# marlbenchmark/off-policy

Hardware: NVIDIA B200
Metric: learner grad-steps/sec (higher is better)
Workload: dtype f32

## Files before the change

### off-policy_b200/csrc/agent_bwd.cu

```cuda
#include "mx_internal.h"
#include "mx_kernels.h"
#include "mx_tile.cuh"
#include "mx_mma.cuh"

static inline size_t qhead_bwd_smem(int A) { return (size_t)(A * MX_H * 9 + 8 * 32 + 2 * 8 * MX_H + 2 * MX_H) * sizeof(float); }

__global__ void __launch_bounds__(256) k_qhead_bwd(QHeadBwdArgs a) {
  MX_DYN_SMEM(smem);
  const int tid = threadIdx.x, lane = tid & 31, warp = tid >> 5;
  const int A = a.A, AW = A * MX_H;
  float* wq_s = smem;
  float* dw_w = wq_s + AW;
  float* db_w = dw_w + 8 * AW;
  float* dg_w = db_w + 8 * 32;
  float* dbt_w = dg_w + 8 * MX_H;
  float* lg_s = dbt_w + 8 * MX_H;
  float* lb_s = lg_s + MX_H;
  for (int i = tid; i < AW; i += blockDim.x) wq_s[i] = a.theta[a.wq + i];
  for (int i = tid; i < 8 * AW + 8 * 32; i += blockDim.x) dw_w[i] = 0.f;
  for (int i = tid; i < MX_H; i += blockDim.x) { lg_s[i] = a.theta[a.lno_g + i]; lb_s[i] = a.theta[a.lno_b + i]; }
  MX_PDL_WAIT();
  __syncthreads();
  const int wglobal = blockIdx.x * (blockDim.x >> 5) + warp;
  const int wtotal = gridDim.x * (blockDim.x >> 5);
// ... 162 lines not shown
      dgh_s[cur][r][sq * MX_H + k] = vs;
      if (dg_on[r]) *dgp[r] = vg;
      dgp[r] -= dg_stride;
      cz[r] = dh * zg;
    }
    mx_cp_wait<PF - 1>();
    __syncthreads();
#pragma unroll
    for (int r = 0; r < RPC; ++r) {
      float2 p0 = make_float2(0.f, 0.f), p1 = p0, p2 = p0;
#pragma unroll
      for (int m = 0; m < 12; m += 3) {
        const float4 d0 = mx_ld4(&dgh_s[cur][r][16 * m + 4 * s]);
        const float4 d1 = mx_ld4(&dgh_s[cur][r][16 * (m + 1) + 4 * s]);
        const float4 d2 = mx_ld4(&dgh_s[cur][r][16 * (m + 2) + 4 * s]);
        p0 = mx_ffma2(w[2 * m], make_float2(d0.x, d0.y), p0); p0 = mx_ffma2(w[2 * m + 1], make_float2(d0.z, d0.w), p0);
        p1 = mx_ffma2(w[2 * m + 2], make_float2(d1.x, d1.y), p1); p1 = mx_ffma2(w[2 * m + 3], make_float2(d1.z, d1.w), p1);
        p2 = mx_ffma2(w[2 * m + 4], make_float2(d2.x, d2.y), p2); p2 = mx_ffma2(w[2 * m + 5], make_float2(d2.z, d2.w), p2);
      }
      p0 = mx_fadd2(mx_fadd2(p0, p1), p2);
      float p = p0.x + p0.y;
      p += __shfl_xor_sync(0xffffffffu, p, 1);
      p += __shfl_xor_sync(0xffffffffu, p, 2);
      carry[r] = cz[r] + p;
    }
  };
  int t = t_first;
  for (; t >= 1; t -= 2) { step(t, 0); step(t - 1, 1); }
  if (t == 0) step(0, 0);
  mx_cp_wait<0>();
}

#define BWD2_THREADS 128
template <int ROWS>
__global__ void __launch_bounds__(BWD2_THREADS, 2) k_gru_bwd2(GruBwdArgs a) {
  constexpr int RING = 8, PF = 6;
  __shared__ __align__(16) float ops_s[RING][ROWS][6][MX_H];
  __shared__ __align__(16) float dgh_s[2][ROWS][MX_G];
  const int tid = threadIdx.x;
  const int kp = tid >> 2, s = tid & 3;
  float2 w0[24], w1[24];
#pragma unroll
  for (int m = 0; m < 12; ++m)
#pragma unroll
    for (int c = 0; c < 2; ++c) {
      const int j = 16 * m + 4 * s + 2 * c;
      w0[2 * m + c] = make_float2(a.theta[a.whh + j * MX_H + 2 * kp], a.theta[a.whh + (j + 1) * MX_H + 2 * kp]);
      w1[2 * m + c] = make_float2(a.theta[a.whh + j * MX_H + 2 * kp + 1], a.theta[a.whh + (j + 1) * MX_H + 2 * kp + 1]);
    }
  const int T1 = a.T1 > 0 ? a.T1 : a.T + 1, N = a.N;
  MX_PDL_WAIT();
  const int t_first = a.T - 1;
  const bool pf_on = tid < 96;
  const int op = pf_on ? tid / 16 : 0, q4 = tid % 16;
  const bool pf_hprev = op == 4;
  const size_t pf_stride = (size_t)N * (op < 3 ? MX_G : MX_H);
  const int ku = 2 * kp + (s & 1);
  const int half = s >> 1;
  const size_t dg_stride = (size_t)N * MX_G;
  bool rok[ROWS];
  const float* pf_src[ROWS];
  const float* pf_h0[ROWS];
  float* dgp[ROWS];
  float carry[ROWS];
#pragma unroll
  for (int r = 0; r < ROWS; ++r) {
    const int row = blockIdx.x * ROWS + r;
    rok[r] = row < a.R;
    const int rr = rok[r] ? row : 0;
    const size_t m0 = ((size_t)(rr / N) * T1) * N + (rr % N);
    const float* base = op < 3 ? a.gates + m0 * MX_G + op * MX_H + 4 * q4 : (op == 3 ? a.hn : (op == 4 ? a.hall : a.dh_out)) + m0 * MX_H + 4 * q4;
    pf_src[r] = base + (ptrdiff_t)(pf_hprev ? t_first - 1 : t_first) * (ptrdiff_t)pf_stride;
    pf_h0[r] = (pf_hprev && a.h0) ? a.h0 + (size_t)rr * MX_H + 4 * q4 : nullptr;
    if (rok[r])
      for (int tz = a.T; tz < T1; ++tz)
        for (int c = tid; c < MX_G; c += BWD2_THREADS) a.dgi[(m0 + (size_t)tz * N) * MX_G + c] = 0.f;
    dgp[r] = a.dgi + (m0 + (size_t)t_first * N) * MX_G + ku;
    carry[r] = 0.f;
  }
  float* pf_dst = &ops_s[0][0][op][4 * q4];
  auto prefetch = [&](int t) {
    if (t >= 0 && pf_on) {
      const bool first = pf_hprev && t == 0;
#pragma unroll
      for (int r = 0; r < ROWS; ++r) {
        if (rok[r]) mx_cp16z(pf_dst + ((t & (RING - 1)) * ROWS + r) * (6 * MX_H), first ? (pf_h0[r] ? pf_h0[r] : a.hall) : pf_src[r], (first && !pf_h0[r]) ? 0 : 16);
        pf_src[r] -= pf_stride;
      }
    }
    mx_cp_commit();
  };
  if (ROWS > 1) {
    for (int idx = tid; idx < RING * ROWS * 6 * MX_H; idx += BWD2_THREADS) (&ops_s[0][0][0][0])[idx] = 0.f;
    __syncthreads();
  }
#pragma unroll
  for (int d = 0; d < PF; ++d) prefetch(t_first - d);
  mx_cp_wait<PF - 1>();
  __syncthreads();

  auto step = [&](const int t, const int cur) {
    prefetch(t - PF);
    float cz[ROWS];
#pragma unroll
    for (int r = 0; r < ROWS; ++r) {
      const float* o = &ops_s[t & (RING - 1)][r][0][0];
      const float rg = o[ku], zg = o[MX_H + ku], ng = o[2 * MX_H + ku], hn = o[3 * MX_H + ku], hp = o[4 * MX_H + ku];
      const float dh = o[5 * MX_H + ku] + carry[r];
      const float d_n = dh * (1.f - zg) * (1.f - ng * ng);
      const float d_z = dh * (hp - ng) * zg * (1.f - zg);
      const float d_r = d_n * hn * rg * (1.f - rg);
      dgh_s[cur][r][(half ? 2 * MX_H : 0) + ku] = half ? d_n * rg : d_r;
      if (!half) dgh_s[cur][r][MX_H + ku] = d_z;
      if (rok[r]) {
        dgp[r][half ? 2 * MX_H : 0] = half ? d_n : d_r;
        if (!half) dgp[r][MX_H] = d_z;
      }
      dgp[r] -= dg_stride;
      cz[r] = dh * zg;
    }
    mx_cp_wait<PF - 1>();
    __syncthreads();
#pragma unroll
    for (int r = 0; r < ROWS; ++r) {
      float2 a0 = make_float2(0.f, 0.f), a1 = a0, b0 = a0, b1 = a0;
#pragma unroll
      for (int m = 0; m < 12; ++m) {
        const float4 d = mx_ld4(&dgh_s[cur][r][16 * m + 4 * s]);
        const float2 lo = make_float2(d.x, d.y), hi = make_float2(d.z, d.w);
        a0 = mx_ffma2(w0[2 * m], lo, a0); b0 = mx_ffma2(w1[2 * m], lo, b0);
        a1 = mx_ffma2(w0[2 * m + 1], hi, a1); b1 = mx_ffma2(w1[2 * m + 1], hi, b1);
      }
      a0 = mx_fadd2(a0, a1); b0 = mx_fadd2(b0, b1);
      float p0 = a0.x + a0.y, p1 = b0.x + b0.y;
      p0 += __shfl_xor_sync(0xffffffffu, p0, 1); p1 += __shfl_xor_sync(0xffffffffu, p1, 1);
      p0 += __shfl_xor_sync(0xffffffffu, p0, 2); p1 += __shfl_xor_sync(0xffffffffu, p1, 2);
      carry[r] = cz[r] + ((s & 1) ? p1 : p0);
    }
  };
  int t = t_first;
  for (; t >= 1; t -= 2) { step(t, 0); step(t - 1, 1); }
  if (t == 0) step(0, 0);
  mx_cp_wait<0>();
}

struct FrontBwdSmem {
  int ldi, ld64, ldg;
  int o_dgi, o_dgn, o_x, o_hp, o_u, o_da, o_x0, o_xh0, o_dx0, o_wc, o_col, o_stat, o_lnp, total;
};
static FrontBwdSmem front_bwd_smem(int in_dim, int TM, bool gru_ext = false) {
  FrontBwdSmem s;
  const int I64 = mx_round_up(in_dim, 64);
  s.ldi = mx_ld(I64); s.ld64 = mx_ld(64); s.ldg = mx_ld(MX_G);
  int o = 0;
  s.o_dgi = o; o += TM * s.ldg;
  s.o_dgn = o; o += gru_ext ? 0 : TM * s.ld64;
  s.o_x = o; o += TM * s.ld64;
  s.o_hp = o; o += gru_ext ? 0 : TM * s.ld64;
  s.o_u = o; o += TM * s.ld64;
  s.o_da = o; o += TM * s.ld64;
  s.o_x0 = o; o += TM * s.ldi;
  s.o_xh0 = o; o += TM * s.ldi;
  s.o_dx0 = o; o += TM * s.ldi;
  s.o_wc = o; o += 64 * s.ld64;
  s.o_col = o; o += 2 * I64 + 4 * 64;
  s.o_stat = o; o += 3 * TM * 2;
  s.o_lnp = o; o += 4 * 64;
  s.total = o;
  return s;
}

template <int RM>
MX_DEVINL void ln64_bwd_relu(bool act_tanh, float (&v)[RM][4], const float* u_s, int ld, const float* stat , const float* gamma_s,
                             float (&dg)[4], float (&db)[4]) {
  const int tx = threadIdx.x & 15, ty = threadIdx.x >> 4;
#pragma unroll
// ... 380 lines not shown
        const float xs[8] = {x0.x, x0.y, x0.z, x0.w, x1.x, x1.y, x1.z, x1.w};
        const float2 d0 = *reinterpret_cast<const float2*>(dgi_s + r * sm.ldg + 2 * tn);
        const float2 d1 = *reinterpret_cast<const float2*>(dgi_s + r * sm.ldg + MX_H + 2 * tn);
        const float2 d2 = *reinterpret_cast<const float2*>(D2_s + r * ld2);
#pragma unroll
        for (int k = 0; k < 8; ++k) {
          const float2 xx = make_float2(xs[k], xs[k]);
          acc[0][k] = mx_ffma2(d0, xx, acc[0][k]);
          acc[1][k] = mx_ffma2(d1, xx, acc[1][k]);
          acc[2][k] = mx_ffma2(d2, xx, acc[2][k]);
        }
      }
      float* W = gp + (pass ? L.whh : L.wih);
#pragma unroll
      for (int g = 0; g < 3; ++g)
#pragma unroll
        for (int h = 0; h < 2; ++h) {
          float* w = W + (size_t)(64 * g + 2 * tn + h) * MX_H + 8 * tk;
          float4 lo = make_float4(h ? acc[g][0].y : acc[g][0].x, h ? acc[g][1].y : acc[g][1].x, h ? acc[g][2].y : acc[g][2].x, h ? acc[g][3].y : acc[g][3].x);
          float4 hi = make_float4(h ? acc[g][4].y : acc[g][4].x, h ? acc[g][5].y : acc[g][5].x, h ? acc[g][6].y : acc[g][6].x, h ? acc[g][7].y : acc[g][7].x);
          if (accum) {
            const float4 p0 = mx_ld4(w), p1 = mx_ld4(w + 4);
            lo.x += p0.x; lo.y += p0.y; lo.z += p0.z; lo.w += p0.w; hi.x += p1.x; hi.y += p1.y; hi.z += p1.z; hi.w += p1.w;
          }
          mx_st4(w, lo); mx_st4(w + 4, hi);
        }
    }
    mx_colsum(dgi_s, sm.ldg, TM, MX_G, gp + L.bih, accum);
    mx_colsum(dgi_s, sm.ldg, TM, 2 * MX_H, gp + L.bhh, accum);
    mx_colsum(dgn_s, sm.ld64, TM, MX_H, gp + L.bhh + 2 * MX_H, accum);
  }
}

int mx_launch_qhead_bwd(const QHeadBwdArgs& a, int* nparts_used, cudaStream_t s) {
  int grid = mx_ceil_div(a.M, 8 * 4);
  const int cap = mx_num_sms();
  if (grid > cap) grid = cap;
  if (grid < 1) grid = 1;
  const size_t smem = qhead_bwd_smem(a.A);
#if !MX_EMU
  static size_t configured = 0;
  if (smem > 48 * 1024 && smem > configured) {
    if (cudaFuncSetAttribute(k_qhead_bwd, cudaFuncAttributeMaxDynamicSharedMemorySize, (int)smem) != cudaSuccess) { mx_set_error("qhead_bwd: smem %zu too large", smem); return 1; }
    configured = smem;
  }
#endif
  MX_LAUNCH_PDL(k_qhead_bwd, dim3(grid), dim3(256), smem, s, a);
  MX_COUNT();
  MX_MARK("k_qhead_bwd", s);
  *nparts_used = grid;
  return MX_CHECK_LAUNCH("qhead_bwd");
}

__global__ void __launch_bounds__(256) k_mlp_dgi(const float* __restrict__ dq_taken, const int32_t* __restrict__ act_idx, int ld_tn,
                                                 float* __restrict__ dgi, int B, int N) {
  const long long total = (long long)B * 2 * N * MX_G;
  MX_PDL_WAIT();
  for (long long i = (long long)blockIdx.x * blockDim.x + threadIdx.x; i < total; i += (long long)gridDim.x * blockDim.x) {
    const int c = (int)(i % MX_G);
    const long long m = i / MX_G;
    const int n = (int)(m % N);
    const long long bt = m / N;
    const int t = (int)(bt & 1);
    const long long b = bt >> 1;
    float v = 0.f;
    if (t == 0 && c == act_idx[b * ld_tn + n]) v = dq_taken[b * N + n];
// ... 88 lines not shown
  else rc = front_bwd_launch<2, false>(a, nparts_used, s);
  if (rc || !a.wgrad_external) return rc;
  return mx_launch_wgrad_tc(a, *nparts_used, s);
}

bool mx_wgrad_tc_usable(const FrontBwdArgs& a);
bool mx_gru_wgrad_split_usable(const FrontBwdArgs& a) {
  if (!g_mx_gru_wgrad_split || g_mx_front_bwd_mma || a.no_gru || a.skip_wgrad) return false;
  return !mx_front_bwd_tc_usable(a) && !mx_wgrad_tc_usable(a);
}
template <int RM>
static int gru_wgrad_launch(const FrontBwdArgs& a, cudaStream_t s) {
  const int TM = 16 * RM;
  GruWgradSmem sm = gru_wgrad_smem(TM);
  const size_t smem = (size_t)sm.total * sizeof(float) + 16;
  const int ntiles = mx_ceil_div(a.M, TM);
  int grid = mx_num_sms();
  if (grid > ntiles) grid = ntiles;
#if !MX_EMU
  static size_t configured = 0;
  if (smem > configured) { cudaFuncSetAttribute(k_gru_wgrad<RM>, cudaFuncAttributeMaxDynamicSharedMemorySize, (int)smem); configured = smem; }
#endif
  MX_LAUNCH_PDL(k_gru_wgrad<RM>, dim3(grid), dim3(MX_TILE_THREADS), smem, s, a, sm);
  MX_COUNT();
  MX_MARK("k_gru_wgrad", s);
  return MX_CHECK_LAUNCH("gru_wgrad");
}
int mx_launch_gru_wgrad(const FrontBwdArgs& a, cudaStream_t s) {
  const int rm = g_mx_front_bwd_rm ? g_mx_front_bwd_rm : front_bwd_pick_rm(a.M, a.L.in_dim, mx_num_sms(), true);
  if (rm == 3) return gru_wgrad_launch<3>(a, s);
  if (rm == 4) return gru_wgrad_launch<4>(a, s);
  return gru_wgrad_launch<2>(a, s);
}
```

### off-policy_b200/csrc/capi_common.cu

```cuda
#include <stdarg.h>
#include <stdio.h>
#include <string.h>

#include "mx_internal.h"

static thread_local char g_err[512] = "";
long long g_mx_launches = 0;
#if !MX_EMU
int g_mx_pdl = -1;
int g_mx_pdl_rows = 12288;
int g_mx_pdl_auto = 0;
int g_mx_pdl_skip_next = 0;
#endif

int g_mx_p2p_timeout_ms = 10000;
int g_mx_gru_rows = 1;
int g_mx_p2p_ll = 1;
int g_mx_mixer_split = 1;
int g_mx_mixer_split_rm = 0;
int g_mx_overlap = 1;
int g_mx_gru_threads = 0;
int g_mx_side_prio = 0;
int g_mx_hyper_late = 0;
int g_mx_mid_fused = 1;
int g_mx_gru_fwd_rpc = 0;
int g_mx_gru_bwd_rpc = 0;
int g_mx_overlap_rows = 1 << 20;
int mx_set_option_common(const char* name, int value) {
  if (!strcmp(name, "mixer_split")) { g_mx_mixer_split = value; return 0; }
  if (!strcmp(name, "mixer_split_rm")) { g_mx_mixer_split_rm = value; return 0; }
  if (!strcmp(name, "overlap")) { g_mx_overlap = value; return 0; }
  if (!strcmp(name, "overlap_rows")) { g_mx_overlap_rows = value; return 0; }
  if (!strcmp(name, "mid_fused")) { g_mx_mid_fused = value; return 0; }
  if (!strcmp(name, "optim_fused")) { g_mx_optim_fused = value; return 0; }
  if (!strcmp(name, "side_prio")) { g_mx_side_prio = value; return 0; }
  if (!strcmp(name, "hyper_late")) { g_mx_hyper_late = value; return 0; }
  if (!strcmp(name, "front_bwd_mma")) { g_mx_front_bwd_mma = value; return 0; }
  if (!strcmp(name, "gru_wgrad_split")) { g_mx_gru_wgrad_split = value; return 0; }
  if (!strcmp(name, "p2p_ll")) { g_mx_p2p_ll = value; return 0; }
  if (!strcmp(name, "gru_rows")) { g_mx_gru_rows = value; return 0; }
  if (!strcmp(name, "p2p_timeout_ms")) { g_mx_p2p_timeout_ms = value; return 0; }
#if !MX_EMU
  if (!strcmp(name, "smem_carveout")) { g_mx_smem_carveout = value; return 0; }
#else
  if (!strcmp(name, "smem_carveout")) return 0;
#endif
  if (!strcmp(name, "gather_tma")) { g_mx_gather_tma = value; return 0; }
  if (!strcmp(name, "gru_threads")) { g_mx_gru_threads = value; return 0; }
  if (!strcmp(name, "gru_fwd_rpc")) { g_mx_gru_fwd_rpc = value; return 0; }
  if (!strcmp(name, "gru_bwd_rpc")) { g_mx_gru_bwd_rpc = value; return 0; }
  return -1;
}

void mx_set_error(const char* fmt, ...) {
  va_list ap;
  va_start(ap, fmt);
  vsnprintf(g_err, sizeof(g_err), fmt, ap);
  va_end(ap);
}

extern "C" const char* mx_last_error(void) { return g_err; }
extern "C" int mx_abi_version(void) { return MX_ABI_VERSION; }

#define MX_MAX_FENCES 256
#if !MX_EMU
static cudaEvent_t g_fence[MX_MAX_FENCES];
static unsigned char g_fence_set[MX_MAX_FENCES];
#endif
static int g_fence_n = 0;
extern "C" int mx_host_fence_alloc(void) {
  if (g_fence_n >= MX_MAX_FENCES) { mx_set_error("mx_host_fence_alloc: out of fences"); return -1; }
// ... 141 lines not shown
```

### off-policy_b200/csrc/mx_common.cuh

```cuda
#pragma once
#include <stdint.h>

#ifdef MARL_EMU
#include "emu_runtime.h"
#define MX_EMU 1
#define MX_LAUNCH_PDL MX_LAUNCH
#define MX_PDL_WAIT() ((void)0)
#define MX_PDL_THETA_WRITTEN() ((void)0)
#else
#include <cuda_runtime.h>
#define MX_EMU 0
#define MX_LAUNCH(kern, grid, block, smem, stream, ...) kern<<<(grid), (block), (smem), (stream)>>>(__VA_ARGS__)

extern int g_mx_pdl, g_mx_pdl_auto, g_mx_pdl_rows;
extern int g_mx_pdl_skip_next;
#define MX_PDL_THETA_WRITTEN() (g_mx_pdl_skip_next = 1)
#define MX_PDL_WAIT()                                                     \
  do {                                                                    \
    asm volatile("griddepcontrol.wait;" ::: "memory");                    \
    asm volatile("griddepcontrol.launch_dependents;" ::: "memory");       \
  } while (0)
extern int g_mx_smem_carveout;
void mx_prefer_carveout(const void* kern);
template <typename... KArgs, typename... Args>
// ... 83 lines not shown
  unsigned sa = (unsigned)__cvta_generic_to_shared(sdst);
  asm volatile("cp.async.cg.shared.global [%0], [%1], 16;" ::"r"(sa), "l"(gsrc) : "memory");
#endif
}
MX_DEVINL void mx_cp16z(float* sdst, const float* gsrc, int nbytes) {
#if MX_EMU
  if (nbytes) *reinterpret_cast<float4*>(sdst) = *reinterpret_cast<const float4*>(gsrc);
  else *reinterpret_cast<float4*>(sdst) = float4{0.f, 0.f, 0.f, 0.f};
#else
  unsigned sa = (unsigned)__cvta_generic_to_shared(sdst);
  asm volatile("cp.async.cg.shared.global [%0], [%1], 16, %2;" ::"r"(sa), "l"(gsrc), "r"(nbytes) : "memory");
#endif
}
MX_DEVINL void mx_cp4(float* sdst, const float* gsrc) {
#if MX_EMU
  *sdst = *gsrc;
#else
  unsigned sa = (unsigned)__cvta_generic_to_shared(sdst);
  asm volatile("cp.async.ca.shared.global [%0], [%1], 4;" ::"r"(sa), "l"(gsrc) : "memory");
#endif
}
MX_DEVINL void mx_cp_commit() {
#if !MX_EMU
  asm volatile("cp.async.commit_group;" ::: "memory");
#endif
}
template <int N>
MX_DEVINL void mx_cp_wait() {
#if !MX_EMU
  asm volatile("cp.async.wait_group %0;" ::"n"(N) : "memory");
#endif
}

MX_DEVINL float mx_ex2(float x) {
#if MX_EMU
  return exp2f(x);
#else
  float r;
  asm("ex2.approx.ftz.f32 %0, %1;" : "=f"(r) : "f"(x));
  return r;
#endif
}
MX_DEVINL float mx_rcp(float x) {
#if MX_EMU
  return 1.0f / x;
#else
  float r;
  asm("rcp.approx.ftz.f32 %0, %1;" : "=f"(r) : "f"(x));
  return r;
#endif
}
MX_DEVINL float mx_sigmoid_fast(float x) { return mx_rcp(1.0f + mx_ex2(-1.4426950408889634f * x)); }
MX_DEVINL float mx_tanh_fast(float x) { return fmaf(2.0f, mx_rcp(1.0f + mx_ex2(-2.8853900817779268f * x)), -1.0f); }

MX_DEVINL float2 mx_ffma2(float2 a, float2 b, float2 c) {
#if MX_EMU
  return make_float2(fmaf(a.x, b.x, c.x), fmaf(a.y, b.y, c.y));
#else
  return __ffma2_rn(a, b, c);
#endif
}
MX_DEVINL float2 mx_fadd2(float2 a, float2 b) {
#if MX_EMU
  return make_float2(a.x + b.x, a.y + b.y);
#else
  return __fadd2_rn(a, b);
// ... 5 lines not shown
```

### off-policy_b200/csrc/mx_internal.h

```cpp
#pragma once
#include "../../include/marl_b200.h"
#include "mx_common.cuh"

#include <functional>
#include <string>

void mx_set_error(const char* fmt, ...);
extern long long g_mx_launches;
extern int g_mx_prof_on;
void mx_prof_mark(const char* name, cudaStream_t s);
extern int g_mx_mixer_split, g_mx_mixer_split_rm, g_mx_overlap, g_mx_overlap_rows, g_mx_mid_fused, g_mx_gru_fwd_rpc, g_mx_gru_bwd_rpc, g_mx_optim_fused, g_mx_gru_threads, g_mx_front_bwd_mma, g_mx_hyper_late, g_mx_side_prio, g_mx_gru_wgrad_split, g_mx_p2p_ll, g_mx_p2p_timeout_ms, g_mx_gru_rows;
int mx_set_option_common(const char* name, int value);
#define MX_COUNT() (++g_mx_launches)
#define MX_MARK(name, s) do { if (g_mx_prof_on) mx_prof_mark((name), (s)); } while (0)

#if MX_EMU
static inline int mx_num_sms() { return 4; }
#define MX_CHECK_LAUNCH(what) 0
#else
int mx_num_sms();
int mx_check_launch(const char* what);
#define MX_CHECK_LAUNCH(what) mx_check_launch(what)
#endif

struct mx_graph {
#if !MX_EMU
  cudaGraph_t graph = nullptr;
  cudaGraphExec_t exec = nullptr;
#endif
  std::function<int(void*)> seq;
  std::function<void()> after_launch;
  int n_kernels = 0;
};
int mx_graph_capture_seq(std::function<int(void*)> seq, std::function<void()> after_launch, void* stream, mx_graph** out);

struct MxReplayState {
  int32_t filled;
  int32_t cursor;
  int32_t rng_pos;
  int32_t pad;
  double max_priority;
  double reward_mean, reward_std;
  double per_beta;
};
// ... 90 lines not shown
```

### off-policy_b200/csrc/mx_kernels.h

```cpp
#pragma once
#include "mx_internal.h"

struct FrontFwdArgs {
  const float* X;
  int ldx, M;
  int feature_norm;
  const float* theta[2];
  MxNetLayout L;
  float* gi[2];
  float *u1, *u2;
  float *st0, *st1, *st2;
  const float* tc_img[2];
  int act_tanh;
};
size_t mx_tc_image_floats(int in_dim);
int mx_launch_tc_prep_weights(const float* const theta[2], const MxNetLayout& L, float* const img[2], int nets, cudaStream_t s);
size_t mx_front_fwd_smem(int in_dim, int RM);
int mx_launch_front_fwd(const FrontFwdArgs& a, int nets, cudaStream_t s);

int mx_launch_pack_prev_act(const float* obs, int obs_ld, const float* acts, int act_ld, float* X, int ldx, int B, int T, int N, int O, int A,
                            cudaStream_t s);

struct GruFwdArgs {
  const float* theta[2];
// ... 115 lines not shown
  const float* X;
  int ldx, M, T, N;
  int T1;
  const float* h0;
  int feature_norm;
  const float* theta;
  MxNetLayout L;
  const float *u1, *u2, *st0, *st1, *st2;
  const float* dgi;
  const float* gates;
  const float* hall;
  float* gpart;
  long long P;
  int no_gru;
  float* dX;
  int skip_wgrad;
  float *da2_out, *da1_out;
  int wgrad_external;
  int use_mma;
  float* tc_imgT;
  int tc_imgT_ready;
  int act_tanh;
  float* ln_part;
  int ln_part_rows;
  int gru_wgrad_ext;
};
bool mx_gru_wgrad_split_usable(const FrontBwdArgs& a);
int mx_launch_gru_wgrad(const FrontBwdArgs& a, cudaStream_t s);
int mx_launch_tc_prep_weights_T(const float* theta, const MxNetLayout& L, float* imgT, cudaStream_t s);
bool mx_tc_prep_T_wanted(int in_dim);
size_t mx_tc_imageT_floats(int in_dim);
int mx_launch_front_bwd(const FrontBwdArgs& a, int* nparts_used, cudaStream_t s);
int mx_launch_wgrad_tc(const FrontBwdArgs& a, int nparts, cudaStream_t s);
bool mx_wgrad_tc_usable(const FrontBwdArgs& a);

struct OptimArgs {
  float *theta, *theta_tgt, *adam_m, *adam_v;
  const float* gpart;
  float* grad;
  long long P;
  int seg_begin[4], seg_end[4], seg_parts[4], nseg;
  const float* spart;
  int spart_n;
  float* info;
  double* adam_t;
  const float* err;
  int B, T;
  float per_nu, per_eps;
  float* prio;
  float lr, beta1, beta2, eps, max_grad_norm, tau;
  int world_size;
  float* normpart;
  int normpart_n;
  int fuse_polyak;
  float weight_decay;
  unsigned* sync;
  int phase;
  float* p2p_blocks[16];
  unsigned long long p2p_timeout_ns;
  int p2p_ll;
  float* xstat;
  long long p2p_slot;
  int p2p_rank, p2p_world;
};
static inline int mx_grad_reduce_blocks(long long P) { return (int)((P + 255) / 256); }
int mx_launch_grad_reduce(const OptimArgs& a, cudaStream_t s);
// ... 5 lines not shown
```

### off-policy_b200/csrc/qmix.cu

```cuda
#include <stdio.h>
#include <string.h>

#include <string>
#include <vector>

#include "mx_internal.h"
#include "mx_kernels.h"

extern int g_mx_front_tc;
bool mx_front_tc_usable(int in_dim, bool have_image);

static int take(int& off, int n) { int o = off; off += mx_round_up(n, 4); return o; }

int mx_net_layout(int in_dim, int out_dim, int base, MxNetLayout* L) {
  const int H = MX_H;
  int o = base;
  L->in_dim = in_dim; L->out_dim = out_dim;
  L->fn_g = take(o, in_dim); L->fn_b = take(o, in_dim);
  L->w1 = take(o, H * in_dim); L->b1 = take(o, H); L->ln1_g = take(o, H); L->ln1_b = take(o, H);
  L->wh = take(o, H * H); L->bh = take(o, H); L->lnh_g = take(o, H); L->lnh_b = take(o, H);
  L->w2 = take(o, H * H); L->b2 = take(o, H); L->ln2_g = take(o, H); L->ln2_b = take(o, H);
  L->wih = take(o, 3 * H * H); L->whh = take(o, 3 * H * H); L->bih = take(o, 3 * H); L->bhh = take(o, 3 * H);
  L->lno_g = take(o, H); L->lno_b = take(o, H);
  L->wq = take(o, out_dim * H); L->bq = take(o, out_dim);
// ... 431 lines not shown
    parts[3] = parts[1];
#if !MX_EMU
    if (overlap) fork_to_side(q, q->ev_core, s);
#endif
    if (mx_launch_mix_hyper_bwd(mx, &parts[2], side)) return 1;
  } else {
    if (mx_launch_qhead(qh, s)) return 1;
    if (split) {
      if (!overlap) { if (mx_launch_mix_hyper_fwd(mx, s)) return 1; }
#if !MX_EMU
      else join_from_side(q, q->ev_hyper, s);
#endif
      if (mx_launch_mix_core(mx, &parts[3], s)) return 1;
#if !MX_EMU
      if (overlap) fork_to_side(q, q->ev_core, s);
#endif
      if (mx_launch_mix_hyper_bwd(mx, &parts[2], side)) return 1;
    } else {
      if (mx_launch_mixer(mx, &parts[2], s)) return 1;
      parts[3] = parts[2];
    }
    QHeadBwdArgs hb;
    memset(&hb, 0, sizeof(hb));
    hb.theta = q->theta; hb.wq = q->agent.wq; hb.bq = q->agent.bq; hb.lno_g = q->agent.lno_g; hb.lno_b = q->agent.lno_b;
    hb.hall = gf.hall[0]; hb.sto = qh.sto; hb.act_idx = b->act_idx; hb.dq_taken = mx.dq_taken;
    hb.M = M; hb.T = T; hb.N = N; hb.A = c.act_dim; hb.ld_tn = ld_tn; hb.dh_out = ws + W.dh_out; hb.gpart = mx.gpart; hb.P = q->P;
    if (mx_launch_qhead_bwd(hb, &parts[1], s)) return 1;
  }

  GruBwdArgs gb;
  memset(&gb, 0, sizeof(gb));
  gb.theta = q->theta; gb.whh = q->agent.whh; gb.hall = gf.hall[0]; gb.gates = gf.gates; gb.hn = gf.hn; gb.dh_out = ws + W.dh_out;
  gb.dgi = ws + W.dgi; gb.R = B * N; gb.T = T; gb.N = N;
  if (mx_launch_gru_bwd(gb, s)) return 1;

  FrontBwdArgs fb;
  memset(&fb, 0, sizeof(fb));
  fb.X = X; fb.ldx = ldx; fb.M = M; fb.T = T; fb.N = N; fb.feature_norm = c.no_feature_norm ? 0 : 1; fb.act_tanh = c.use_tanh;
  fb.theta = q->theta; fb.L = q->agent; fb.u1 = ff.u1; fb.u2 = ff.u2; fb.st0 = ff.st0; fb.st1 = ff.st1; fb.st2 = ff.st2;
  fb.dgi = gb.dgi; fb.gates = gf.gates; fb.hall = gf.hall[0]; fb.gpart = mx.gpart; fb.P = q->P;
  fb.ln_part = ws + W.lnpart; fb.ln_part_rows = 2 * q->npart;
  fb.da2_out = ws + W.da2; fb.da1_out = ws + W.da1; fb.tc_imgT = ws + W.tcimgT; fb.tc_imgT_ready = q->imgT_fresh; q->imgT_fresh = 0;
  const bool gsplit = mx_gru_wgrad_split_usable(fb);
  if (gsplit) {
    fb.gru_wgrad_ext = 1;
#if !MX_EMU
    if (overlap) fork_to_side(q, q->ev_gbwd, s);
#endif
    if (mx_launch_gru_wgrad(fb, side)) return 1;
  }
  if (mx_launch_front_bwd(fb, &parts[0], s)) return 1;

#if !MX_EMU
  if ((split || gsplit) && overlap) join_from_side(q, q->ev_hbwd, s);
#endif
  *oa = optim_args(q, B, parts);
  return 0;
}

extern "C" int mx_qmix_backward_only(mx_qmix* q, const mx_batch* b, void* stream) {
  OptimArgs o;
  if (backward_core(q, b, stream, &o)) return 1;
  return mx_launch_grad_reduce(o, (cudaStream_t)stream);
}

extern "C" int mx_qmix_apply_ex(mx_qmix* q, uint32_t flags, void* stream) {
  const int parts[4] = {0, 0, 0, 0};
  OptimArgs o = optim_args(q, q->cfg.max_batch, parts, true);
  o.fuse_polyak = (flags & MX_STEP_FUSE_SOFT_UPDATE) ? 1 : 0;
  return mx_launch_adam(o, (cudaStream_t)stream);
}
extern "C" int mx_qmix_apply(mx_qmix* q, void* stream) { return mx_qmix_apply_ex(q, 0, stream); }

extern "C" int mx_qmix_step_ex(mx_qmix* q, const mx_batch* b, uint32_t flags, void* stream) {
  OptimArgs o;
  if (backward_core(q, b, stream, &o)) return 1;
  if (q->cfg.world_size == 1 || q->p2p_world) {
    o.fuse_polyak = (flags & MX_STEP_FUSE_SOFT_UPDATE) ? 1 : 0;
    const int rc = mx_launch_optim_fused(o, (cudaStream_t)stream);
    if (rc >= 0) return rc;
  }
  if (mx_launch_grad_reduce(o, (cudaStream_t)stream)) return 1;
  if (q->cfg.world_size > 1) {
    if (!q->p2p_world) return 0;
// ... 95 lines not shown
```

Baseline: 5935.

## Fuse GRU backward recurrence with front backward via warp-specialized producer/consumer kernel

Adds a fused kernel where one 128-thread group runs the reverse GRU recurrence per row and writes gate gradients into a double-buffered shared-memory chunk. A 256-thread consumer group computes the input-side weight grads, LN backward and MLP backward on each 16-step chunk as it completes. The two groups coordinate through named barriers. This removes the dgi round trip through global memory and one launch, and overlaps the serial recurrence with the front backward work. The fused path needs one block per row with the row count at most the SM count, and it disables the side-stream wgrad split when it is taken.

```diff
diff --git a/off-policy_b200/csrc/agent_bwd.cu b/off-policy_b200/csrc/agent_bwd.cu
--- a/off-policy_b200/csrc/agent_bwd.cu
+++ b/off-policy_b200/csrc/agent_bwd.cu
@@ -218,14 +218,13 @@
 }
 
 #define BWD2_THREADS 128
-template <int ROWS>
-__global__ void __launch_bounds__(BWD2_THREADS, 2) k_gru_bwd2(GruBwdArgs a) {
-  constexpr int RING = 8, PF = 6;
-  __shared__ __align__(16) float ops_s[RING][ROWS][6][MX_H];
-  __shared__ __align__(16) float dgh_s[2][ROWS][MX_G];
-  const int tid = threadIdx.x;
+struct GruBwdNoHook {
+  MX_DEVINL void begin(int) const {}
+  MX_DEVINL void value(int, int, int, float, float, float) const {}
+  MX_DEVINL void end(int) const {}
+};
+MX_DEVINL void gru_bwd2_load_w(const GruBwdArgs& a, int tid, float2 (&w0)[24], float2 (&w1)[24]) {
   const int kp = tid >> 2, s = tid & 3;
-  float2 w0[24], w1[24];
 #pragma unroll
   for (int m = 0; m < 12; ++m)
 #pragma unroll
@@ -234,8 +233,13 @@
       w0[2 * m + c] = make_float2(a.theta[a.whh + j * MX_H + 2 * kp], a.theta[a.whh + (j + 1) * MX_H + 2 * kp]);
       w1[2 * m + c] = make_float2(a.theta[a.whh + j * MX_H + 2 * kp + 1], a.theta[a.whh + (j + 1) * MX_H + 2 * kp + 1]);
     }
+}
+template <int ROWS, class Sync, class Hook>
+MX_DEVINL void gru_bwd2_body(const GruBwdArgs& a, const int tid, const int row_base, const float2 (&w0)[24], const float2 (&w1)[24],
+                             float (*ops_s)[ROWS][6][MX_H], float (*dgh_s)[ROWS][MX_G], Sync sync, const Hook& hook) {
+  constexpr int RING = 8, PF = 6;
+  const int kp = tid >> 2, s = tid & 3;
   const int T1 = a.T1 > 0 ? a.T1 : a.T + 1, N = a.N;
-  MX_PDL_WAIT();
   const int t_first = a.T - 1;
   const bool pf_on = tid < 96;
   const int op = pf_on ? tid / 16 : 0, q4 = tid % 16;
@@ -251,7 +255,7 @@
   float carry[ROWS];
 #pragma unroll
   for (int r = 0; r < ROWS; ++r) {
-    const int row = blockIdx.x * ROWS + r;
+    const int row = row_base + r;
     rok[r] = row < a.R;
     const int rr = rok[r] ? row : 0;
     const size_t m0 = ((size_t)(rr / N) * T1) * N + (rr % N);
@@ -278,14 +282,15 @@
   };
   if (ROWS > 1) {
     for (int idx = tid; idx < RING * ROWS * 6 * MX_H; idx += BWD2_THREADS) (&ops_s[0][0][0][0])[idx] = 0.f;
-    __syncthreads();
+    sync();
   }
 #pragma unroll
   for (int d = 0; d < PF; ++d) prefetch(t_first - d);
   mx_cp_wait<PF - 1>();
-  __syncthreads();
+  sync();
 
   auto step = [&](const int t, const int cur) {
+    hook.begin(t);
     prefetch(t - PF);
     float cz[ROWS];
 #pragma unroll
@@ -302,11 +307,13 @@
         dgp[r][half ? 2 * MX_H : 0] = half ? d_n : d_r;
         if (!half) dgp[r][MX_H] = d_z;
       }
+      hook.value(t, ku, half, d_r, d_z, d_n);
       dgp[r] -= dg_stride;
       cz[r] = dh * zg;
     }
+    hook.end(t);
     mx_cp_wait<PF - 1>();
-    __syncthreads();
+    sync();
 #pragma unroll
     for (int r = 0; r < ROWS; ++r) {
       float2 a0 = make_float2(0.f, 0.f), a1 = a0, b0 = a0, b1 = a0;
@@ -328,6 +335,18 @@
   for (; t >= 1; t -= 2) { step(t, 0); step(t - 1, 1); }
   if (t == 0) step(0, 0);
   mx_cp_wait<0>();
+}
+
+struct BlockSync { MX_DEVINL void operator()() const { __syncthreads(); } };
+
+template <int ROWS>
+__global__ void __launch_bounds__(BWD2_THREADS, 2) k_gru_bwd2(GruBwdArgs a) {
+  __shared__ __align__(16) float ops_s[8][ROWS][6][MX_H];
+  __shared__ __align__(16) float dgh_s[2][ROWS][MX_G];
+  float2 w0[24], w1[24];
+  gru_bwd2_load_w(a, threadIdx.x, w0, w1);
+  MX_PDL_WAIT();
+  gru_bwd2_body<ROWS>(a, threadIdx.x, blockIdx.x * ROWS, w0, w1, ops_s, dgh_s, BlockSync(), GruBwdNoHook());
 }
 
 struct FrontBwdSmem {
@@ -774,6 +793,201 @@
   }
 }
 
+#define BF_CONSUMERS 256
+#define BF_THREADS (BF_CONSUMERS + BWD2_THREADS)
+#define BF_TC 16
+#define BF_BAR_REC 1
+#define BF_BAR_FRONT 2
+#define BF_BAR_FULL 3
+#define BF_BAR_EMPTY 5
+
+struct BwdFrontSmem { int ld64, ldg, o_dgi, o_wih, o_w2, o_w1, o_dgn, o_x, o_hp, o_u2, o_u1, o_da, o_x0, o_xh0, o_stat, o_lnp, o_col, o_ops, o_dgh, total; };
+static BwdFrontSmem bwd_front_smem() {
+  BwdFrontSmem s;
+  s.ld64 = mx_ld(64); s.ldg = mx_ld(MX_G);
+  int o = 0;
+  s.o_dgi = o; o += 2 * BF_TC * s.ldg;
+  s.o_wih = o; o += MX_G * s.ld64;
+  s.o_w2 = o; o += MX_H * s.ld64;
+  s.o_w1 = o; o += MX_H * s.ld64;
+  s.o_dgn = o; o += BF_TC * s.ld64;
+  s.o_x = o; o += BF_TC * s.ld64;
+  s.o_hp = o; o += BF_TC * s.ld64;
+  s.o_u2 = o; o += BF_TC * s.ld64;
+  s.o_u1 = o; o += BF_TC * s.ld64;
+  s.o_da = o; o += BF_TC * s.ld64;
+  s.o_x0 = o; o += BF_TC * s.ld64;
+  s.o_xh0 = o; o += BF_TC * s.ld64;
+  s.o_stat = o; o += 3 * BF_TC * 2;
+  s.o_lnp = o; o += 4 * 64;
+  s.o_col = o; o += 6 * 64;
+  s.o_ops = o; o += 8 * 6 * MX_H;
+  s.o_dgh = o; o += 2 * MX_G;
+  s.total = o;
+  return s;
+}
+
+struct RecSync { MX_DEVINL void operator()() const { mx_bar_sync(BF_BAR_REC, BWD2_THREADS); } };
+struct BwdFrontHook {
+  float* dgi_s;
+  int ldg, T;
+  MX_DEVINL int chunk(int t) const { return (T - 1 - t) / BF_TC; }
+  MX_DEVINL int t_lo(int c) const { return mx_imax(0, T - BF_TC * (c + 1)); }
+  MX_DEVINL void begin(int t) const {
+    const int c = chunk(t);
+    if (c >= 2 && t == T - 1 - BF_TC * c) mx_bar_sync(BF_BAR_EMPTY + (c & 1), BF_THREADS);
+  }
+  MX_DEVINL void value(int t, int ku, int half, float d_r, float d_z, float d_n) const {
+    const int c = chunk(t);
+    float* row = dgi_s + ((c & 1) * BF_TC + (t - t_lo(c))) * ldg;
+    if (half) row[2 * MX_H + ku] = d_n;
+    else { row[ku] = d_r; row[MX_H + ku] = d_z; }
+  }
+  MX_DEVINL void end(int t) const {
+    const int c = chunk(t);
+    if (t == t_lo(c)) mx_bar_arrive(BF_BAR_FULL + (c & 1), BF_THREADS);
+  }
+};
+
+__global__ void __launch_bounds__(BF_THREADS, 1) k_gru_bwd_front(GruBwdArgs g, FrontBwdArgs a, BwdFrontSmem sm) {
+  MX_DYN_SMEM(smem);
+  const int tid = threadIdx.x, row = blockIdx.x;
+  const int T = g.T, nchunks = (T + BF_TC - 1) / BF_TC;
+  const int ld64 = sm.ld64, ldg = sm.ldg;
+  float* dgi_s = smem + sm.o_dgi;
+  if (tid >= BF_CONSUMERS) {
+    const int rt = tid - BF_CONSUMERS;
+    float2 w0[24], w1[24];
+    gru_bwd2_load_w(g, rt, w0, w1);
+    MX_PDL_WAIT();
+    BwdFrontHook hook;
+    hook.dgi_s = dgi_s; hook.ldg = ldg; hook.T = T;
+    gru_bwd2_body<1>(g, rt, row, w0, w1, reinterpret_cast<float (*)[1][6][MX_H]>(smem + sm.o_ops),
+                     reinterpret_cast<float (*)[1][MX_G]>(smem + sm.o_dgh), RecSync(), hook);
+    return;
+  }
+  const MxNetLayout L = a.L;
+  const float* __restrict__ th = a.theta;
+  const int I = L.in_dim, tx = tid & 15, ty = tid >> 4;
+  float* wih_s = smem + sm.o_wih; float* w2_s = smem + sm.o_w2; float* w1_s = smem + sm.o_w1;
+  float* dgn_s = smem + sm.o_dgn; float* x_s = smem + sm.o_x; float* hp_s = smem + sm.o_hp;
+  float* u2_s = smem + sm.o_u2; float* u1_s = smem + sm.o_u1; float* da_s = smem + sm.o_da;
+  float* x0_s = smem + sm.o_x0; float* xh0_s = smem + sm.o_xh0;
+  float* st0_s = smem + sm.o_stat; float* st1_s = st0_s + 2 * BF_TC; float* st2_s = st1_s + 2 * BF_TC;
+  float* ln1g_s = smem + sm.o_lnp; float* ln1b_s = ln1g_s + 64; float* ln2g_s = ln1b_s + 64; float* ln2b_s = ln2g_s + 64;
+  float* col0g = smem + sm.o_col; float* col0b = col0g + 64; float* col1g = col0b + 64; float* col1b = col1g + 64;
+  float* col2g = col1b + 64; float* col2b = col2g + 64;
+  for (int nc = 0; nc < 3; ++nc) mx_stage_weight(wih_s + nc * 64 * ld64, ld64, th + L.wih, MX_G, MX_H, MX_H, nc * 64, 0, 64, false);
+  mx_stage_weight(w2_s, ld64, th + L.w2, MX_H, MX_H, MX_H, 0, 0, 64, false);
+  mx_stage_weight(w1_s, ld64, th + L.w1, MX_H, I, I, 0, 0, 64, false);
+  for (int i = tid; i < 6 * 64; i += BF_CONSUMERS) col0g[i] = 0.f;
+  if (tid < 64) { ln1g_s[tid] = th[L.ln1_g + tid]; ln1b_s[tid] = th[L.ln1_b + tid]; ln2g_s[tid] = th[L.ln2_g + tid]; ln2b_s[tid] = th[L.ln2_b + tid]; }
+  MX_PDL_WAIT();
+  const int T1 = g.T1 > 0 ? g.T1 : T + 1, N = g.N;
+  const size_t mrow = ((size_t)(row / N) * T1) * N + (row % N);
+  const bool ldx_vec = (a.ldx & 3) == 0;
+  float* gp = a.gpart + (size_t)row * a.P;
+  float dg1[4] = {0.f, 0.f, 0.f, 0.f}, db1[4] = {0.f, 0.f, 0.f, 0.f}, dg2[4] = {0.f, 0.f, 0.f, 0.f}, db2[4] = {0.f, 0.f, 0.f, 0.f};
+  float cg[4] = {0.f, 0.f, 0.f, 0.f}, cb[4] = {0.f, 0.f, 0.f, 0.f};
+  for (int c = 0; c < nchunks; ++c) {
+    const int t_lo = mx_imax(0, T - BF_TC * (c + 1)), len = T - BF_TC * c - t_lo;
+    const size_t mb = mrow + (size_t)t_lo * N;
+    const bool accum = c > 0;
+    float* dgi_c = dgi_s + (c & 1) * BF_TC * ldg;
+    mx_stage_rows(dgn_s, ld64, a.gates + mb * MX_G, (size_t)N * MX_G, 0, len, BF_TC, MX_H);
+    mx_stage_rows(u2_s, ld64, a.u2 + mb * MX_H, (size_t)N * MX_H, 0, len, BF_TC, MX_H);
+    mx_stage_rows(u1_s, ld64, a.u1 + mb * MX_H, (size_t)N * MX_H, 0, len, BF_TC, MX_H);
+    for (int r = ty; r < BF_TC; r += BF_CONSUMERS / 16) {
+      float* d = hp_s + r * ld64 + 4 * tx;
+      if (r < len && t_lo + r > 0) mx_cp16(d, a.hall + (mb + (size_t)r * N - N) * MX_H + 4 * tx);
+      else mx_st4(d, make_float4(0.f, 0.f, 0.f, 0.f));
+    }
+    if (ldx_vec) mx_stage_rows(x0_s, ld64, a.X + mb * a.ldx, (size_t)N * a.ldx, 0, len, BF_TC, mx_round_up(I, 4));
+    mx_cp_commit();
+    for (int i = tid; i < 3 * BF_TC * 2; i += BF_CONSUMERS) {
+      const int which = i / (2 * BF_TC), rr = (i % (2 * BF_TC)) >> 1, comp = i & 1;
+      const float* src = which == 0 ? a.st0 : (which == 1 ? a.st1 : a.st2);
+      st0_s[i] = (rr < len && (which > 0 || a.feature_norm)) ? src[2 * (mb + (size_t)rr * N) + comp] : 0.f;
+    }
+    mx_bar_sync(BF_BAR_FULL + (c & 1), BF_THREADS);
+    for (int i = len * MX_G + tid; i < BF_TC * MX_G; i += BF_CONSUMERS) dgi_c[(i / MX_G) * ldg + i % MX_G] = 0.f;
+    mx_cp_wait<0>();
+    mx_bar_sync(BF_BAR_FRONT, BF_CONSUMERS);
+    for (int idx = tid; idx < BF_TC * MX_H; idx += BF_CONSUMERS) {
+      const int r = idx >> 6, cc = idx & 63;
+      const int o = r * ld64 + cc;
+      dgn_s[o] = dgi_c[r * ldg + 2 * MX_H + cc] * dgn_s[o];
+      x_s[o] = r < len ? (u2_s[o] - st2_s[2 * r]) * st2_s[2 * r + 1] * ln2g_s[cc] + ln2b_s[cc] : 0.f;
+    }
+    mx_bar_sync(BF_BAR_FRONT, BF_CONSUMERS);
+    for (int nb = 0; nb < 3; ++nb) {
+      mx_wgrad_block(dgi_c + nb * 64, ldg, x_s, ld64, len, gp + L.wih, MX_G, MX_H, nb * 64, 0, accum);
+      mx_wgrad_block(nb < 2 ? dgi_c + nb * 64 : dgn_s, nb < 2 ? ldg : ld64, hp_s, ld64, len, gp + L.whh + nb * 64 * MX_H, 64, MX_H, 0, 0, accum);
+    }
+    mx_colsum(dgi_c, ldg, len, MX_G, gp + L.bih, accum);
+    mx_colsum(dgi_c, ldg, len, 2 * MX_H, gp + L.bhh, accum);
+    mx_colsum(dgn_s, ld64, len, MX_H, gp + L.bhh + 2 * MX_H, accum);
+    float v[1][4] = {{0.f, 0.f, 0.f, 0.f}};
+    for (int nc = 0; nc < 3; ++nc) mx_mm_nn<1>(dgi_c + nc * 64, ldg, wih_s + nc * 64 * ld64, ld64, v);
+    if (c + 2 < nchunks) mx_bar_arrive(BF_BAR_EMPTY + (c & 1), BF_THREADS);
+    ln64_bwd_relu<1>(a.act_tanh != 0, v, u2_s, ld64, st2_s, ln2g_s, dg2, db2);
+    mx_bar_sync(BF_BAR_FRONT, BF_CONSUMERS);
+    mx_st4(da_s + ty * ld64 + 4 * tx, make_float4(v[0][0], v[0][1], v[0][2], v[0][3]));
+    for (int idx = tid; idx < BF_TC * MX_H; idx += BF_CONSUMERS) {
+      const int r = idx >> 6, cc = idx & 63;
+      const int o = r * ld64 + cc;
+      x_s[o] = r < len ? (u1_s[o] - st1_s[2 * r]) * st1_s[2 * r + 1] * ln1g_s[cc] + ln1b_s[cc] : 0.f;
+    }
+    mx_bar_sync(BF_BAR_FRONT, BF_CONSUMERS);
+    mx_wgrad_block(da_s, ld64, x_s, ld64, len, gp + L.w2, MX_H, MX_H, 0, 0, accum);
+    mx_colsum(da_s, ld64, len, MX_H, gp + L.b2, accum);
+    v[0][0] = v[0][1] = v[0][2] = v[0][3] = 0.f;
+    mx_mm_nn<1>(da_s, ld64, w2_s, ld64, v);
+    ln64_bwd_relu<1>(a.act_tanh != 0, v, u1_s, ld64, st1_s, ln1g_s, dg1, db1);
+    mx_bar_sync(BF_BAR_FRONT, BF_CONSUMERS);
+    mx_st4(da_s + ty * ld64 + 4 * tx, make_float4(v[0][0], v[0][1], v[0][2], v[0][3]));
+    for (int idx = tid; idx < BF_TC * 64; idx += BF_CONSUMERS) {
+      const int r = idx >> 6, cc = idx & 63;
+      float xh = 0.f, x0 = 0.f;
+      if (r < len && cc < I) {
+        const float x = ldx_vec ? x0_s[r * ld64 + cc] : a.X[(mb + (size_t)r * N) * a.ldx + cc];
+        if (a.feature_norm) {
+          xh = (x - st0_s[2 * r]) * st0_s[2 * r + 1];
+          x0 = xh * th[L.fn_g + cc] + th[L.fn_b + cc];
+        } else x0 = x;
+      }
+      x0_s[r * ld64 + cc] = x0; xh0_s[r * ld64 + cc] = xh;
+    }
+    mx_bar_sync(BF_BAR_FRONT, BF_CONSUMERS);
+    mx_wgrad_block(da_s, ld64, x0_s, ld64, len, gp + L.w1, MX_H, I, 0, 0, accum);
+    mx_colsum(da_s, ld64, len, MX_H, gp + L.b1, accum);
+    if (a.feature_norm) {
+      v[0][0] = v[0][1] = v[0][2] = v[0][3] = 0.f;
+      mx_mm_nn<1>(da_s, ld64, w1_s, ld64, v);
+#pragma unroll
+      for (int jx = 0; jx < 4; ++jx) { cg[jx] = fmaf(v[0][jx], xh0_s[ty * ld64 + 4 * tx + jx], cg[jx]); cb[jx] += v[0][jx]; }
+    }
+    mx_bar_sync(BF_BAR_FRONT, BF_CONSUMERS);
+  }
+  for (int grp = 0; grp < BF_CONSUMERS / 16; ++grp) {
+    if (ty == grp) {
+#pragma unroll
+      for (int jx = 0; jx < 4; ++jx) {
+        const int cc = 4 * tx + jx;
+        col0g[cc] += cg[jx]; col0b[cc] += cb[jx];
+        col1g[cc] += dg1[jx]; col1b[cc] += db1[jx];
+        col2g[cc] += dg2[jx]; col2b[cc] += db2[jx];
+      }
+    }
+    mx_bar_sync(BF_BAR_FRONT, BF_CONSUMERS);
+  }
+  if (tid < MX_H) {
+    gp[L.ln2_g + tid] = col2g[tid]; gp[L.ln2_b + tid] = col2b[tid];
+    gp[L.ln1_g + tid] = col1g[tid]; gp[L.ln1_b + tid] = col1b[tid];
+    if (tid < I) { gp[L.fn_g + tid] = col0g[tid]; gp[L.fn_b + tid] = col0b[tid]; }
+  }
+}
+
 int mx_launch_qhead_bwd(const QHeadBwdArgs& a, int* nparts_used, cudaStream_t s) {
   int grid = mx_ceil_div(a.M, 8 * 4);
   const int cap = mx_num_sms();
@@ -928,3 +1142,24 @@
   if (rm == 4) return gru_wgrad_launch<4>(a, s);
   return gru_wgrad_launch<2>(a, s);
 }
+
+int g_mx_bwd_fused = -1;
+bool mx_gru_bwd_front_usable(const GruBwdArgs& g, const FrontBwdArgs& a, int nparts, bool debug) {
+  if (g_mx_bwd_fused == 0 || (g_mx_bwd_fused < 0 && debug)) return false;
+  if (a.no_gru || a.skip_wgrad || a.dX || g.h0 || a.h0 || g.T1 || a.T1 || g.T < 1 || a.L.in_dim > 64) return false;
+  if (g_mx_gru_threads == 256 || g_mx_front_bwd_mma || mx_front_bwd_tc_usable(a) || mx_wgrad_tc_usable(a)) return false;
+  return g.R <= nparts && g.R <= mx_num_sms();
+}
+int mx_launch_gru_bwd_front(const GruBwdArgs& g, const FrontBwdArgs& a, int* nparts_used, cudaStream_t s) {
+  const BwdFrontSmem sm = bwd_front_smem();
+  const size_t smem = (size_t)sm.total * sizeof(float) + 16;
+#if !MX_EMU
+  static bool configured = false;
+  if (!configured) { cudaFuncSetAttribute(k_gru_bwd_front, cudaFuncAttributeMaxDynamicSharedMemorySize, (int)smem); configured = true; }
+#endif
+  MX_LAUNCH_PDL(k_gru_bwd_front, dim3(g.R), dim3(BF_THREADS), smem, s, g, a, sm);
+  MX_COUNT();
+  MX_MARK("k_gru_bwd_front", s);
+  *nparts_used = g.R;
+  return MX_CHECK_LAUNCH("gru_bwd_front");
+}
diff --git a/off-policy_b200/csrc/capi_common.cu b/off-policy_b200/csrc/capi_common.cu
--- a/off-policy_b200/csrc/capi_common.cu
+++ b/off-policy_b200/csrc/capi_common.cu
@@ -37,6 +37,7 @@
   if (!strcmp(name, "hyper_late")) { g_mx_hyper_late = value; return 0; }
   if (!strcmp(name, "front_bwd_mma")) { g_mx_front_bwd_mma = value; return 0; }
   if (!strcmp(name, "gru_wgrad_split")) { g_mx_gru_wgrad_split = value; return 0; }
+  if (!strcmp(name, "bwd_fused")) { g_mx_bwd_fused = value; return 0; }
   if (!strcmp(name, "p2p_ll")) { g_mx_p2p_ll = value; return 0; }
   if (!strcmp(name, "gru_rows")) { g_mx_gru_rows = value; return 0; }
   if (!strcmp(name, "p2p_timeout_ms")) { g_mx_p2p_timeout_ms = value; return 0; }
diff --git a/off-policy_b200/csrc/mx_common.cuh b/off-policy_b200/csrc/mx_common.cuh
--- a/off-policy_b200/csrc/mx_common.cuh
+++ b/off-policy_b200/csrc/mx_common.cuh
@@ -139,6 +139,36 @@
 #endif
 }
 
+#if MX_EMU
+namespace mx_emu_bar {
+inline int arrived[16], gen[16];
+inline bool count(int id, int n) {
+  if (id < 1 || id >= 16 || n <= 0 || n % 32 != 0 || n > emu::g.nthreads) { fprintf(stderr, "emu: bad named barrier %d / %d threads\n", id, n); abort(); }
+  if (++arrived[id] < n) return false;
+  arrived[id] = 0;
+  gen[id]++;
+  emu::g.progress++;
+  return true;
+}
+}
+#endif
+MX_DEVINL void mx_bar_sync(int id, int nthreads) {
+#if MX_EMU
+  const int gen = mx_emu_bar::gen[id];
+  if (!mx_emu_bar::count(id, nthreads))
+    while (mx_emu_bar::gen[id] == gen) emu::yield();
+#else
+  asm volatile("bar.sync %0, %1;" ::"r"(id), "r"(nthreads) : "memory");
+#endif
+}
+MX_DEVINL void mx_bar_arrive(int id, int nthreads) {
+#if MX_EMU
+  mx_emu_bar::count(id, nthreads);
+#else
+  asm volatile("bar.arrive %0, %1;" ::"r"(id), "r"(nthreads) : "memory");
+#endif
+}
+
 MX_DEVINL float mx_ex2(float x) {
 #if MX_EMU
   return exp2f(x);
diff --git a/off-policy_b200/csrc/mx_internal.h b/off-policy_b200/csrc/mx_internal.h
--- a/off-policy_b200/csrc/mx_internal.h
+++ b/off-policy_b200/csrc/mx_internal.h
@@ -9,7 +9,7 @@
 extern long long g_mx_launches;
 extern int g_mx_prof_on;
 void mx_prof_mark(const char* name, cudaStream_t s);
-extern int g_mx_mixer_split, g_mx_mixer_split_rm, g_mx_overlap, g_mx_overlap_rows, g_mx_mid_fused, g_mx_gru_fwd_rpc, g_mx_gru_bwd_rpc, g_mx_optim_fused, g_mx_gru_threads, g_mx_front_bwd_mma, g_mx_hyper_late, g_mx_side_prio, g_mx_gru_wgrad_split, g_mx_p2p_ll, g_mx_p2p_timeout_ms, g_mx_gru_rows;
+extern int g_mx_mixer_split, g_mx_mixer_split_rm, g_mx_overlap, g_mx_overlap_rows, g_mx_mid_fused, g_mx_gru_fwd_rpc, g_mx_gru_bwd_rpc, g_mx_optim_fused, g_mx_gru_threads, g_mx_front_bwd_mma, g_mx_hyper_late, g_mx_side_prio, g_mx_gru_wgrad_split, g_mx_p2p_ll, g_mx_p2p_timeout_ms, g_mx_gru_rows, g_mx_bwd_fused;
 int mx_set_option_common(const char* name, int value);
 #define MX_COUNT() (++g_mx_launches)
 #define MX_MARK(name, s) do { if (g_mx_prof_on) mx_prof_mark((name), (s)); } while (0)
diff --git a/off-policy_b200/csrc/mx_kernels.h b/off-policy_b200/csrc/mx_kernels.h
--- a/off-policy_b200/csrc/mx_kernels.h
+++ b/off-policy_b200/csrc/mx_kernels.h
@@ -171,6 +171,8 @@
 size_t mx_tc_imageT_floats(int in_dim);
 int mx_launch_front_bwd(const FrontBwdArgs& a, int* nparts_used, cudaStream_t s);
 int mx_launch_wgrad_tc(const FrontBwdArgs& a, int nparts, cudaStream_t s);
+bool mx_gru_bwd_front_usable(const GruBwdArgs& g, const FrontBwdArgs& a, int nparts, bool debug);
+int mx_launch_gru_bwd_front(const GruBwdArgs& g, const FrontBwdArgs& a, int* nparts_used, cudaStream_t s);
 bool mx_wgrad_tc_usable(const FrontBwdArgs& a);
 
 struct OptimArgs {
diff --git a/off-policy_b200/csrc/qmix.cu b/off-policy_b200/csrc/qmix.cu
--- a/off-policy_b200/csrc/qmix.cu
+++ b/off-policy_b200/csrc/qmix.cu
@@ -487,7 +487,6 @@
   memset(&gb, 0, sizeof(gb));
   gb.theta = q->theta; gb.whh = q->agent.whh; gb.hall = gf.hall[0]; gb.gates = gf.gates; gb.hn = gf.hn; gb.dh_out = ws + W.dh_out;
   gb.dgi = ws + W.dgi; gb.R = B * N; gb.T = T; gb.N = N;
-  if (mx_launch_gru_bwd(gb, s)) return 1;
 
   FrontBwdArgs fb;
   memset(&fb, 0, sizeof(fb));
@@ -496,15 +495,21 @@
   fb.dgi = gb.dgi; fb.gates = gf.gates; fb.hall = gf.hall[0]; fb.gpart = mx.gpart; fb.P = q->P;
   fb.ln_part = ws + W.lnpart; fb.ln_part_rows = 2 * q->npart;
   fb.da2_out = ws + W.da2; fb.da1_out = ws + W.da1; fb.tc_imgT = ws + W.tcimgT; fb.tc_imgT_ready = q->imgT_fresh; q->imgT_fresh = 0;
-  const bool gsplit = mx_gru_wgrad_split_usable(fb);
-  if (gsplit) {
-    fb.gru_wgrad_ext = 1;
-#if !MX_EMU
-    if (overlap) fork_to_side(q, q->ev_gbwd, s);
-#endif
-    if (mx_launch_gru_wgrad(fb, side)) return 1;
-  }
-  if (mx_launch_front_bwd(fb, &parts[0], s)) return 1;
+  bool gsplit = false;
+  if (mx_gru_bwd_front_usable(gb, fb, q->npart, q->debug != 0)) {
+    if (mx_launch_gru_bwd_front(gb, fb, &parts[0], s)) return 1;
+  } else {
+    if (mx_launch_gru_bwd(gb, s)) return 1;
+    gsplit = mx_gru_wgrad_split_usable(fb);
+    if (gsplit) {
+      fb.gru_wgrad_ext = 1;
+#if !MX_EMU
+      if (overlap) fork_to_side(q, q->ev_gbwd, s);
+#endif
+      if (mx_launch_gru_wgrad(fb, side)) return 1;
+    }
+    if (mx_launch_front_bwd(fb, &parts[0], s)) return 1;
+  }
 
 #if !MX_EMU
   if ((split || gsplit) && overlap) join_from_side(q, q->ev_hbwd, s);
```

Result: slower. 5067, median of 6 (-14.6%).
